# OnurBasci/TransformerBasedNavierStokeSolver

Measured on AMD Instinct MI355X. Metric: ns64_train_samples_per_s, higher is better.
Workload: dtype f32

## Files before the change

### transformerbasednavierstokesolver_amd/csrc/pa2d_gemm.hip

```cpp
#include "pa2d_gemm_common.h"
#include <string.h>


static Pa2dEnv read_env() {
    auto is = [](const char* n, const char* pre) { const char* e = getenv(n); return e && strncmp(e, pre, strlen(pre)) == 0; };
    auto num = [](const char* n, int dflt) { const char* e = getenv(n); return (e && e[0]) ? atoi(e) : dflt; };
    Pa2dEnv v;
    v.conv_halo = is("PA2D_CONV_HALO", "o") ? 0 : (is("PA2D_CONV_HALO", "f") ? 2 : 1);
    v.mc_big_off = is("PA2D_MC_BIG", "o") ? 1 : 0;
    v.kc_bk16 = num("PA2D_KC_BK", 0) == 16 ? 1 : 0;
    v.mc_bk = num("PA2D_MC_BK", 16) == 32 ? 32 : 16;
    v.mc_splits = num("PA2D_MC_SPLITS", 0);
    v.mcb_splits = num("PA2D_MCB_SPLITS", 0);
    v.lin_dw_split = is("PA2D_LIN_DW_SPLIT", "of") ? 0 : 1;
    v.lin_panel = is("PA2D_LIN_PANEL", "of") ? 0 : 1;
    v.lin_rowpanel = is("PA2D_LIN_ROWPANEL", "of") ? 0 : 1;
    v.lin_small_split = is("PA2D_LIN_SMALL_SPLIT", "of") ? 0 : 1;
    v.conv_mfma16 = num("PA2D_CONV_MFMA", 16) == 32 ? 0 : 1;
    v.split_big = num("PA2D_SPLIT_BIG", 1);
    v.slice_map = is("PA2D_SLICE_MAP", "l") ? 0 : 1;
    v.default_engine = is("PA2D_GEMM", "f") ? 0 : (is("PA2D_GEMM", "b") ? 2 : 1);
    return v;
}
static Pa2dEnv g_env = read_env();
const Pa2dEnv& pa2d_env() { return g_env; }
static int kc_bk(bool im2col, int Cin) {
    if (im2col && pa2d_env().kc_bk16) return 16;
    return (!im2col || (Cin % 32) == 0) ? 32 : 16;
}
KCTile kc_tile(int M, int N, bool im2col, int Cin) {
    const int tiles_m = ceil_div(M, 128);
    const long long t128 = (long long)tiles_m * ceil_div(N, 128);
    const long long t12864 = (long long)tiles_m * ceil_div(N, 64);
    const int bk = kc_bk(im2col, Cin);
    if (N > 64 && t128 >= 384) return {128, 128, bk};
    if (t12864 >= 384 || M <= 64) return {128, 64, bk};
    return {64, 64, bk};
}
bool use_split(int engine, int N, bool im2col, int Cin) {
    const int m = engine;
    if (m == 1) return im2col && N > 64 && (Cin % 32) == 0;
    if (m == 2) return N > 64 && (!im2col || (Cin % 32) == 0);
    return false;
}

int launch_kc(const KCParams& p_in, bool im2col, hipStream_t st, hipEvent_t ev0, hipEvent_t ev1) {
    KCParams p = p_in;
    if (!engine_ok(p.engine)) return PA2D_ERR_ARG;
    if (p.M <= 0 || p.N <= 0 || p.K <= 0) return PA2D_OK;
    if (!p.bias2) p.bias_split = 0x7fffffff;
    {
        const unsigned long long ab = ((unsigned long long)(p.M - 1) * p.lda + (im2col ? p.Cin : p.K)) * 4ull;
        const unsigned long long bb = ((unsigned long long)(p.N - 1) * p.ldb + p.K) * 4ull;
        if (ab >= 0xFFFFFFF0ull || bb >= 0xFFFFFFF0ull) return PA2D_ERR_UNSUPPORTED;
        p.a_bytes = (unsigned)ab;
        p.b_bytes = (unsigned)bb;
        const unsigned long long es = p.io_bf16 ? 2ull : 4ull;
        const unsigned long long cb = ((unsigned long long)(p.M - 1) * p.ldc + p.N) * es;
        const unsigned long long rb = p.res ? ((unsigned long long)(p.M - 1) * p.ldres + p.N) * es : 0ull;
        const unsigned long long xb = p.aux ? ((unsigned long long)(p.M - 1) * p.ldaux + p.N) * es : 0ull;
        if (cb >= 0xFFFFFFF0ull || rb >= 0xFFFFFFF0ull || xb >= 0xFFFFFFF0ull) return PA2D_ERR_UNSUPPORTED;
        p.c_bytes = (unsigned)cb; p.res_bytes = (unsigned)rb; p.aux_bytes = (unsigned)xb;
    }
    if ((p.K & 3) || (p.lda & 3) || (p.ldb & 3)) return PA2D_ERR_ARG;
    if (im2col && ((p.Cin & 15) || p.K != (p.taps == 27 ? 27 : 9) * p.Cin)) return PA2D_ERR_UNSUPPORTED;
    if (im2col && (p.epi != 0 || p.res)) return PA2D_ERR_ARG;
    if (ev0 && hipEventRecord(ev0, st) != hipSuccess) return PA2D_ERR_ARG;
    int rc;
    if (!im2col && p.wimg && rowpanel_applies(p)) {
        if (p.wsrc) {
            rc = launch_pack_weight_image(p.wsrc, p.wsn, p.wsk, p.wimg, p.N, p.K, st);
            if (rc) return rc;
        }
        KCParams pp = p;
        pp.M = p.M - p.M % 128;
        rc = launch_kc_rowpanel(pp, p.wimg, st);
        if (!rc && pp.M < p.M) {
            KCParams pt = p_in;
            pt.wimg = nullptr;
            pt.M = p.M - pp.M;
            pt.A = p.A + (size_t)pp.M * p.lda;
            pt.C = p.C + (size_t)pp.M * p.ldc;
            if (p.res) pt.res = p.res + (size_t)pp.M * p.ldres;
            if (p.aux) pt.aux = p.aux + (size_t)pp.M * p.ldaux;
            rc = launch_kc(pt, false, st);
        }
    } else if (panel_applies(p, im2col)) {
        KCParams pp = p;
        pp.M = p.M - p.M % 256;
        rc = launch_kc_panel(pp, st);
        if (!rc && pp.M < p.M) {
            KCParams pt = p_in;
            const size_t ea = p.io_bf16 ? 2 : 4, es = p.io_bf16 ? 2 : 4;
            pt.M = p.M - pp.M;
            pt.A = (const float*)((const char*)p.A + (size_t)pp.M * p.lda * ea);
            pt.C = (float*)((char*)p.C + (size_t)pp.M * p.ldc * es);
            if (p.res) pt.res = (const float*)((const char*)p.res + (size_t)pp.M * p.ldres * es);
            if (p.aux) pt.aux = (float*)((char*)p.aux + (size_t)pp.M * p.ldaux * es);
            rc = launch_kc(pt, false, st);
        }
    } else if (p.io_bf16 || use_split(p.engine, p.N, im2col, p.Cin)) rc = launch_kc_split(p, im2col, st);
// ... 198 lines not shown
```

### transformerbasednavierstokesolver_amd/csrc/pa2d_gemm_mc_planes.hip

```cpp
#include "pa2d_gemm_common.h"
#include "pa2d_bf16_split.h"

struct MCPlanesParams {
    const void* PA; int chA;
    const void* PB; int chB;
    float* slab;
    int Mi, Nj, Mk, chunks_per_split, splits, H, W, Cin;
    unsigned a_bytes, b_bytes;
    int taps;
    long long lda, ldb;
    float* colsum;
};

__device__ __forceinline__ unsigned img_off(int row, int ch) {
    return 256u * row + 16u * (ch ^ (((row & 3) << 2) | ((row >> 2) & 3)));
}

template <int NT, int KS, bool F32SRC = false>
__global__ __launch_bounds__(256, 2) void gemm_mc_planes_kernel(const MCPlanesParams p) {
    constexpr int PIMG = 4096;
    constexpr int STAGE = 2 * NT * KS * PIMG;
    constexpr int NP = 2 * NT * KS;
    __shared__ __attribute__((aligned(16))) unsigned char smem[2 * STAGE];

    const int tid = threadIdx.x, lane = tid & 63, wave = tid >> 6;
    const int tiles_i = (p.Mi + 127) / 128, tiles_j = (p.Nj + 127) / 128;
    int tj, ti, split;
    {
        const int tiles = tiles_i * tiles_j;
        if ((p.splits & 7) == 0) {
            const int xcd = blockIdx.x & 7, slot = blockIdx.x >> 3, q = p.splits >> 3;
            split = xcd * q + slot / tiles;
            const int t = slot % tiles;
            tj = t % tiles_j;
            ti = t / tiles_j;
        } else {
            tj = blockIdx.x % tiles_j;
            ti = (blockIdx.x / tiles_j) % tiles_i;
            split = blockIdx.x / tiles;
        }
    }
    const int wm = wave >> 1, wn = wave & 1;
    const int total_chunks = (p.Mk + 15) / 16;
    const int c_begin = split * p.chunks_per_split;
    const int c_end = min(total_chunks, c_begin + p.chunks_per_split);

    const int j0 = tj * 128, tap = j0 / p.Cin, cb0 = (j0 - tap * p.Cin) >> 5, ca0 = (ti * 128) >> 5;
    const int tap_dy = tap / 3 - 1, tap_dx = tap - (tap / 3) * 3 - 1, tap_shift = tap_dy * p.W + tap_dx;
    const int HW = p.H * p.W;

    const __amdgpu_buffer_rsrc_t ra_rsrc = __builtin_amdgcn_make_buffer_rsrc(const_cast<void*>(p.PA), 0, p.a_bytes, 0x00020000);
    const __amdgpu_buffer_rsrc_t rb_rsrc = __builtin_amdgcn_make_buffer_rsrc(const_cast<void*>(p.PB), 0, p.b_bytes, 0x00020000);

    int s_row[NP];
    unsigned s_goff[NP], s_lds[NP];
    bool s_isb[NP];
#pragma unroll
    for (int s = 0; s < NP; ++s) {
        const int q = tid + 256 * s;
        const int op = q / (256 * NT * KS), r = q - op * (256 * NT * KS);
        const int row = r / (16 * NT), rr = r - row * (16 * NT);
        const int c = rr / (4 * NT), pp = rr - c * (4 * NT);
        const int plane = pp >> 2, piece = pp & 3;
        s_row[s] = row;
        s_isb[s] = op != 0;
        s_goff[s] = (unsigned)((((op ? cb0 : ca0) + c) * NT + plane) * 64 + piece * 16);
        s_lds[s] = (unsigned)(((op * NT + plane) * KS + (row >> 4)) * PIMG) + img_off(row & 15, c * 4 + piece);
    }
    u32x4 rg[F32SRC ? 4 * KS : NP];
    const int frow = tid >> 4, fc8 = tid & 15;
    const unsigned flds = img_off(frow, fc8);
    const bool fok_a = ti * 128 + fc8 * 8 < p.Mi, fok_b = tj * 128 + fc8 * 8 < p.Nj;
    const unsigned fcol_a = (unsigned)(ti * 128 + fc8 * 8) * 4u, fcol_b = (unsigned)(tj * 128 + fc8 * 8) * 4u;
    const unsigned fpitch_a = (unsigned)p.lda * 4u, fpitch_b = (unsigned)p.ldb * 4u;
    float cs[8];
#pragma unroll
    for (int e = 0; e < 8; ++e) cs[e] = 0.f;
#define MP_LOAD(c_)                                                                                       \
    if constexpr (F32SRC) {                                                                               \
        _Pragma("unroll") for (int ks = 0; ks < KS; ++ks) {                                               \
            const int m_ = ((c_) + ks) * 16 + frow;                                                       \
            const bool okr_ = m_ < p.Mk && (c_) + ks < c_end;                                             \
            const unsigned oa_ = (okr_ && fok_a) ? (unsigned)m_ * fpitch_a + fcol_a : OOB_OFF;            \
            const unsigned ob_ = (okr_ && fok_b) ? (unsigned)m_ * fpitch_b + fcol_b : OOB_OFF;            \
            rg[ks * 4 + 0] = __builtin_amdgcn_raw_buffer_load_b128(ra_rsrc, oa_, 0, 0);                   \
            rg[ks * 4 + 1] = __builtin_amdgcn_raw_buffer_load_b128(ra_rsrc, oa_ == OOB_OFF ? OOB_OFF : oa_ + 16u, 0, 0); \
            rg[ks * 4 + 2] = __builtin_amdgcn_raw_buffer_load_b128(rb_rsrc, ob_, 0, 0);                   \
            rg[ks * 4 + 3] = __builtin_amdgcn_raw_buffer_load_b128(rb_rsrc, ob_ == OOB_OFF ? OOB_OFF : ob_ + 16u, 0, 0); \
        }                                                                                                 \
    } else {                                                                                              \
        const int m0_ = (c_) * 16;                                                                        \
        _Pragma("unroll") for (int s = 0; s < NP; ++s) {                                                  \
            const int m_ = m0_ + s_row[s];                                                                \
            bool ok_ = m_ < p.Mk && (KS == 1 || (c_) + (s_row[s] >> 4) < c_end);    \
            int mm_ = m_;                                                                                 \
            if (s_isb[s]) {                                                                               \
                const int n_ = m_ % HW;                                                                   \
                const int y_ = n_ / p.W, x_ = n_ - y_ * p.W;                                              \
                ok_ = ok_ && (unsigned)(y_ + tap_dy) < (unsigned)p.H && (unsigned)(x_ + tap_dx) < (unsigned)p.W; \
                mm_ = m_ + tap_shift;                                                                     \
            }                                                                                             \
            const unsigned rowb_ = (unsigned)mm_ * (unsigned)((s_isb[s] ? p.chB : p.chA) * NT * 64);      \
            rg[s] = s_isb[s] ? __builtin_amdgcn_raw_buffer_load_b128(rb_rsrc, ok_ ? rowb_ + s_goff[s] : OOB_OFF, 0, 0) \
                             : __builtin_amdgcn_raw_buffer_load_b128(ra_rsrc, ok_ ? rowb_ + s_goff[s] : OOB_OFF, 0, 0); \
        }                                                                                                 \
    }
#define MP_STORE(buf_)                                                                                    \
    if constexpr (F32SRC) {                                                                               \
        _Pragma("unroll") for (int ks = 0; ks < KS; ++ks) _Pragma("unroll") for (int op = 0; op < 2; ++op) { \
            const u32x4 u0_ = rg[ks * 4 + op * 2], u1_ = rg[ks * 4 + op * 2 + 1];                         \
            const float4 v0_ = make_float4(__uint_as_float(u0_.x), __uint_as_float(u0_.y), __uint_as_float(u0_.z), __uint_as_float(u0_.w)); \
            const float4 v1_ = make_float4(__uint_as_float(u1_.x), __uint_as_float(u1_.y), __uint_as_float(u1_.z), __uint_as_float(u1_.w)); \
            if (op == 0 && do_cs) {                                                                       \
                cs[0] += v0_.x; cs[1] += v0_.y; cs[2] += v0_.z; cs[3] += v0_.w;                           \
                cs[4] += v1_.x; cs[5] += v1_.y; cs[6] += v1_.z; cs[7] += v1_.w;                           \
            }                                                                                             \
            bf16x4 h0_, m0_, l0_, h1_, m1_, l1_;                                                          \
            split3(v0_, h0_, m0_, l0_);                                                                   \
            split3(v1_, h1_, m1_, l1_);                                                                   \
            unsigned char* d_ = smem + (buf_) * STAGE + flds;                                             \
            *reinterpret_cast<bf16x8*>(d_ + ((op * NT + 0) * KS + ks) * PIMG) = __builtin_shufflevector(h0_, h1_, 0, 1, 2, 3, 4, 5, 6, 7); \
            if (NT == 3) {                                                                                \
                *reinterpret_cast<bf16x8*>(d_ + ((op * NT + 1) * KS + ks) * PIMG) = __builtin_shufflevector(m0_, m1_, 0, 1, 2, 3, 4, 5, 6, 7); \
                *reinterpret_cast<bf16x8*>(d_ + ((op * NT + 2) * KS + ks) * PIMG) = __builtin_shufflevector(l0_, l1_, 0, 1, 2, 3, 4, 5, 6, 7); \
            }                                                                                             \
        }                                                                                                 \
    } else {                                                                                              \
        _Pragma("unroll") for (int s = 0; s < NP; ++s)                                                    \
            *reinterpret_cast<u32x4*>(smem + (buf_) * STAGE + s_lds[s]) = rg[s];                          \
    }
    const bool do_cs = F32SRC && p.colsum != nullptr && tj == 0;

    f32x16 acc[2][2];
#pragma unroll
    for (int i = 0; i < 2; ++i)
#pragma unroll
        for (int j = 0; j < 2; ++j)
#pragma unroll
            for (int r = 0; r < 16; ++r) acc[i][j][r] = 0.f;

    const int g = lane >> 4, q4 = (lane & 15) >> 2, pq = lane & 3;
    unsigned fa[2][2], fb[2][2];
#pragma unroll
    for (int t = 0; t < 2; ++t)
#pragma unroll
        for (int r = 0; r < 2; ++r) {
            const int row = 8 * (g >> 1) + 4 * r + q4;
            const int cha = ((wm * 64 + t * 32) >> 3) + 2 * (g & 1) + (pq >> 1);
            const int chb = ((wn * 64 + t * 32) >> 3) + 2 * (g & 1) + (pq >> 1);
            fa[t][r] = img_off(row, cha) + 8u * (pq & 1);
            fb[t][r] = img_off(row, chb) + 8u * (pq & 1);
        }

    if (c_begin < c_end) {
        MP_LOAD(c_begin)
        MP_STORE(0)
    }
    __syncthreads();
    for (int c = c_begin; c < c_end; c += KS) {
        const int buf = ((c - c_begin) / KS) & 1;
        if (c + KS < c_end) { MP_LOAD(c + KS) }
#pragma unroll
        for (int ks = 0; ks < KS; ++ks) {
        const unsigned char* st = smem + buf * STAGE + ks * PIMG;
        bf16x8 af[2][NT], bf[2][NT];
#pragma unroll
        for (int t = 0; t < 2; ++t)
#pragma unroll
            for (int pl = 0; pl < NT; ++pl) {
                typedef __attribute__((address_space(3))) s16x4 lds_s16x4;
                const s16x4 a0 = __builtin_amdgcn_ds_read_tr16_b64_v4i16((lds_s16x4*)(st + pl * KS * PIMG + fa[t][0]));
                const s16x4 a1 = __builtin_amdgcn_ds_read_tr16_b64_v4i16((lds_s16x4*)(st + pl * KS * PIMG + fa[t][1]));
                const s16x4 b0 = __builtin_amdgcn_ds_read_tr16_b64_v4i16((lds_s16x4*)(st + (NT + pl) * KS * PIMG + fb[t][0]));
                const s16x4 b1 = __builtin_amdgcn_ds_read_tr16_b64_v4i16((lds_s16x4*)(st + (NT + pl) * KS * PIMG + fb[t][1]));
                const s16x8 av = __builtin_shufflevector(a0, a1, 0, 1, 2, 3, 4, 5, 6, 7);
                const s16x8 bv = __builtin_shufflevector(b0, b1, 0, 1, 2, 3, 4, 5, 6, 7);
                af[t][pl] = __builtin_bit_cast(bf16x8, av);
                bf[t][pl] = __builtin_bit_cast(bf16x8, bv);
            }
#pragma unroll
        for (int i = 0; i < 2; ++i)
#pragma unroll
            for (int j = 0; j < 2; ++j) {
                if constexpr (NT == 3) {
                    acc[i][j] = __builtin_amdgcn_mfma_f32_32x32x16_bf16(af[i][1], bf[j][1], acc[i][j], 0, 0, 0);
                    acc[i][j] = __builtin_amdgcn_mfma_f32_32x32x16_bf16(af[i][2], bf[j][0], acc[i][j], 0, 0, 0);
                    acc[i][j] = __builtin_amdgcn_mfma_f32_32x32x16_bf16(af[i][0], bf[j][2], acc[i][j], 0, 0, 0);
                    acc[i][j] = __builtin_amdgcn_mfma_f32_32x32x16_bf16(af[i][1], bf[j][0], acc[i][j], 0, 0, 0);
                    acc[i][j] = __builtin_amdgcn_mfma_f32_32x32x16_bf16(af[i][0], bf[j][1], acc[i][j], 0, 0, 0);
                }
                acc[i][j] = __builtin_amdgcn_mfma_f32_32x32x16_bf16(af[i][0], bf[j][0], acc[i][j], 0, 0, 0);
            }
        }
        if (c + KS < c_end) { MP_STORE(buf ^ 1) }
        __syncthreads();
    }
#undef MP_LOAD
#undef MP_STORE

    if constexpr (F32SRC) {
        if (do_cs) {
            float* sm = reinterpret_cast<float*>(smem);
#pragma unroll
            for (int e = 0; e < 8; ++e) sm[frow * 128 + fc8 * 8 + e] = cs[e];
            __syncthreads();
            if (tid < 128) {
                float t = 0.f;
#pragma unroll
                for (int r = 0; r < 16; ++r) t += sm[r * 128 + tid];
                if (ti * 128 + tid < p.Mi) p.colsum[(size_t)split * p.Mi + ti * 128 + tid] = t;
            }
        }
    }
    float* out = p.slab + (size_t)split * p.Mi * p.Nj;
    const int col0 = tj * 128 + wn * 64 + (lane & 31);
    const int row0 = ti * 128 + wm * 64 + 4 * (lane >> 5);
#pragma unroll
    for (int j = 0; j < 2; ++j)
#pragma unroll
        for (int i = 0; i < 2; ++i)
#pragma unroll
            for (int r = 0; r < 16; ++r) {
                const int row = row0 + i * 32 + (r & 3) + 8 * (r >> 2);
                if (!F32SRC || (row < p.Mi && col0 + j * 32 < p.Nj)) out[(size_t)row * p.Nj + col0 + j * 32] = acc[i][j][r];
            }
}

bool mc_planes_supported(int C, int Cin) { return (C % 64) == 0 && (Cin % 128) == 0; }

int launch_mc_planes(const void* PA, const void* PB, int C, int Cin, int Mk, int H, int W, float* slab,
                     const MCPlan& pl, int NT, hipStream_t st) {
    if (!mc_planes_supported(C, Cin) || !pl.big) return PA2D_ERR_UNSUPPORTED;
    MCPlanesParams p;
    p.PA = PA; p.chA = 2 * C / 32; p.PB = PB; p.chB = Cin / 32; p.slab = slab;
    p.Mi = 2 * C; p.Nj = 9 * Cin; p.Mk = Mk; p.chunks_per_split = pl.chunks_per_split; p.splits = pl.splits;
    p.H = H; p.W = W; p.Cin = Cin; p.taps = 9;
    const unsigned long long ab = (unsigned long long)Mk * p.chA * NT * 64, bb = (unsigned long long)Mk * p.chB * NT * 64;
    if (ab >= 0xFFFFFFF0ull || bb >= 0xFFFFFFF0ull) return PA2D_ERR_UNSUPPORTED;
    p.a_bytes = (unsigned)ab; p.b_bytes = (unsigned)bb;
    const dim3 grid((p.Mi / 128) * (p.Nj / 128) * pl.splits);
    if (NT == 3) hipLaunchKernelGGL((gemm_mc_planes_kernel<3, 1>), grid, dim3(256), 0, st, p);
    else hipLaunchKernelGGL((gemm_mc_planes_kernel<1, 4>), grid, dim3(256), 0, st, p);
    PA2D_CHECK_LAUNCH();
    return PA2D_OK;
}

template <int NT, int KS>
__global__ __launch_bounds__(512, 1) void gemm_mc_planes_big_kernel(const MCPlanesParams p, const int per_xcd) {
    constexpr int PIMG = 8192;
    constexpr int STAGE = 2 * NT * KS * PIMG;
    constexpr int NP = (2 * NT * KS * 512) / 512;
    extern __shared__ __attribute__((aligned(16))) unsigned char smem[];

    const int tid = threadIdx.x, lane = tid & 63, wave = tid >> 6;
    const int tiles_i = (p.Mi + 255) / 256, tiles_j = (p.Nj + 255) / 256;
    const int tiles = tiles_i * tiles_j;
    const int lin = (blockIdx.x & 7) * per_xcd + (blockIdx.x >> 3);
    if ((int)(blockIdx.x >> 3) >= per_xcd || lin >= tiles * p.splits) return;
    const int split = lin / tiles, t_ = lin - split * tiles;
    const int ti = t_ / tiles_j, tj = t_ - ti * tiles_j;
    const int wm = wave >> 2, wn = wave & 3;
    const int total_chunks = (p.Mk + 15) / 16;
    const int c_begin = split * p.chunks_per_split;
    const int c_end = min(total_chunks, c_begin + p.chunks_per_split);
    const int HW = p.taps == 1 ? 1 : p.H * p.W;

    const __amdgpu_buffer_rsrc_t ra_rsrc = __builtin_amdgcn_make_buffer_rsrc(const_cast<void*>(p.PA), 0, p.a_bytes, 0x00020000);
    const __amdgpu_buffer_rsrc_t rb_rsrc = __builtin_amdgcn_make_buffer_rsrc(const_cast<void*>(p.PB), 0, p.b_bytes, 0x00020000);

    const int row16 = tid >> 5, cgrp = (tid & 31) >> 2, piece = tid & 3;
    const bool colok_a = ti * 256 + cgrp * 32 < p.Mi;
    const unsigned goff_a = (unsigned)((((ti * 256) >> 5) + cgrp) * NT * 64 + piece * 16);
    const int jc = tj * 256 + cgrp * 32;
    const int tap = p.taps == 1 ? 4 : jc / p.Cin;
    const bool colok_b = jc < p.Nj;
    const unsigned goff_b = (unsigned)((p.taps == 1 ? (jc >> 5) : ((jc - tap * p.Cin) >> 5)) * NT * 64 + piece * 16);
    const int tap_dy = tap / 3 - 1, tap_dx = tap - (tap / 3) * 3 - 1, tap_shift = tap_dy * p.W + tap_dx;
    const unsigned pitch_a = (unsigned)(p.chA * NT * 64), pitch_b = (unsigned)(p.chB * NT * 64);
    const unsigned lds_off = 512u * row16 + 16u * ((unsigned)(cgrp * 4 + piece) ^ (unsigned)(((row16 & 3) << 2) | ((row16 >> 2) & 3)));
#define MB_LOAD(c_, RG)                                                                                   \
    {                                                                                                     \
        _Pragma("unroll") for (int ks = 0; ks < KS; ++ks) {                                               \
            const int m_ = ((c_) + ks) * 16 + row16;                                                      \
            const bool okr_ = m_ < p.Mk && (c_) + ks < c_end;             \
            bool okb_ = okr_ && colok_b;                                                                  \
            int mm_ = m_;                                                                                 \
            if (p.taps != 1) {       \
                okb_ = okb_ && (unsigned)(ly + tap_dy) < (unsigned)p.H && (unsigned)(lx + tap_dx) < (unsigned)p.W; \
                mm_ = m_ + tap_shift;                                                                     \
                lx += 16;                                                                                 \
                while (lx >= p.W) { lx -= p.W; ++ly; }                                                    \
                while (ly >= p.H) ly -= p.H;                                                              \
            }                                                                                             \
            const unsigned oa_ = (okr_ && colok_a) ? (unsigned)m_ * pitch_a + goff_a : OOB_OFF;           \
            const unsigned ob_ = okb_ ? (unsigned)mm_ * pitch_b + goff_b : OOB_OFF;                       \
            _Pragma("unroll") for (int pl = 0; pl < NT; ++pl) {                                           \
                RG[pl * KS + ks] = __builtin_amdgcn_raw_buffer_load_b128(ra_rsrc, oa_ == OOB_OFF ? OOB_OFF : oa_ + pl * 64u, 0, 0); \
                RG[(NT + pl) * KS + ks] = __builtin_amdgcn_raw_buffer_load_b128(rb_rsrc, ob_ == OOB_OFF ? OOB_OFF : ob_ + pl * 64u, 0, 0); \
            }                                                                                             \
        }                                                                                                 \
    }
#define MB_STORE(buf_, RG)                                                                                \
    {                                                                                                     \
        _Pragma("unroll") for (int s = 0; s < NP; ++s)                                                    \
            *reinterpret_cast<u32x4*>(smem + (buf_) * STAGE + s * PIMG + lds_off) = RG[s];                \
    }
    u32x4 rg0[NP];
    int ly = 0, lx = 0;
    if (p.taps != 1) {
        const int n0 = (c_begin * 16 + row16) % HW;
        ly = n0 / p.W;
        lx = n0 - ly * p.W;
    }

    f32x16 acc[4][2];
#pragma unroll
    for (int i = 0; i < 4; ++i)
#pragma unroll
        for (int j = 0; j < 2; ++j)
#pragma unroll
            for (int r = 0; r < 16; ++r) acc[i][j][r] = 0.f;

    const int g = lane >> 4, q4 = (lane & 15) >> 2, pq = lane & 3;
    unsigned fa[4][2], fb[2][2];
#pragma unroll
    for (int r = 0; r < 2; ++r) {
        const int row = 8 * (g >> 1) + 4 * r + q4;
        const unsigned swz = (unsigned)(((row & 3) << 2) | ((row >> 2) & 3));
#pragma unroll
        for (int t = 0; t < 4; ++t) {
            const int cha = ((wm * 128 + t * 32) >> 3) + 2 * (g & 1) + (pq >> 1);
            fa[t][r] = 512u * row + 16u * ((unsigned)cha ^ swz) + 8u * (pq & 1);
        }
#pragma unroll
        for (int t = 0; t < 2; ++t) {
            const int chb = ((wn * 64 + t * 32) >> 3) + 2 * (g & 1) + (pq >> 1);
            fb[t][r] = 512u * row + 16u * ((unsigned)chb ^ swz) + 8u * (pq & 1);
        }
    }

#define MB_COMPUTE(buf_)                                                                                  \
    _Pragma("unroll") for (int ks = 0; ks < KS; ++ks) {                                                   \
        const unsigned char* st = smem + (buf_) * STAGE + ks * PIMG;                                      \
        bf16x8 af[4][NT], bf[2][NT];                                                                      \
        typedef __attribute__((address_space(3))) s16x4 lds_s16x4;                                        \
        _Pragma("unroll") for (int pl = 0; pl < NT; ++pl) {                                               \
            _Pragma("unroll") for (int t = 0; t < 4; ++t) {                                               \
                const s16x4 a0 = __builtin_amdgcn_ds_read_tr16_b64_v4i16((lds_s16x4*)(st + pl * KS * PIMG + fa[t][0])); \
                const s16x4 a1 = __builtin_amdgcn_ds_read_tr16_b64_v4i16((lds_s16x4*)(st + pl * KS * PIMG + fa[t][1])); \
                af[t][pl] = __builtin_bit_cast(bf16x8, __builtin_shufflevector(a0, a1, 0, 1, 2, 3, 4, 5, 6, 7)); \
            }                                                                                             \
            _Pragma("unroll") for (int t = 0; t < 2; ++t) {                                               \
                const s16x4 b0 = __builtin_amdgcn_ds_read_tr16_b64_v4i16((lds_s16x4*)(st + (NT + pl) * KS * PIMG + fb[t][0])); \
                const s16x4 b1 = __builtin_amdgcn_ds_read_tr16_b64_v4i16((lds_s16x4*)(st + (NT + pl) * KS * PIMG + fb[t][1])); \
                bf[t][pl] = __builtin_bit_cast(bf16x8, __builtin_shufflevector(b0, b1, 0, 1, 2, 3, 4, 5, 6, 7)); \
            }                                                                                             \
        }                                                                                                 \
        _Pragma("unroll") for (int i = 0; i < 4; ++i)                                                     \
            _Pragma("unroll") for (int j = 0; j < 2; ++j) {                                               \
                if constexpr (NT == 3) {                                        \
                    acc[i][j] = __builtin_amdgcn_mfma_f32_32x32x16_bf16(af[i][1], bf[j][1], acc[i][j], 0, 0, 0); \
                    acc[i][j] = __builtin_amdgcn_mfma_f32_32x32x16_bf16(af[i][2], bf[j][0], acc[i][j], 0, 0, 0); \
                    acc[i][j] = __builtin_amdgcn_mfma_f32_32x32x16_bf16(af[i][0], bf[j][2], acc[i][j], 0, 0, 0); \
                    acc[i][j] = __builtin_amdgcn_mfma_f32_32x32x16_bf16(af[i][1], bf[j][0], acc[i][j], 0, 0, 0); \
                    acc[i][j] = __builtin_amdgcn_mfma_f32_32x32x16_bf16(af[i][0], bf[j][1], acc[i][j], 0, 0, 0); \
                }                                                                                         \
                acc[i][j] = __builtin_amdgcn_mfma_f32_32x32x16_bf16(af[i][0], bf[j][0], acc[i][j], 0, 0, 0); \
            }                                                                                             \
    }
    if (c_begin < c_end) {
        MB_LOAD(c_begin, rg0)
        MB_STORE(0, rg0)
        if (c_begin + KS < c_end) MB_LOAD(c_begin + KS, rg0)
    }
    __syncthreads();
    for (int c = c_begin; c < c_end; c += KS) {
        const int buf = ((c - c_begin) / KS) & 1;
        if (c + KS < c_end) {
            MB_STORE(buf ^ 1, rg0)
            if (c + 2 * KS < c_end) MB_LOAD(c + 2 * KS, rg0)
        }
        MB_COMPUTE(buf)
        __syncthreads();
    }
#undef MB_COMPUTE
#undef MB_LOAD
#undef MB_STORE

    float* out = p.slab + (size_t)split * p.Mi * p.Nj;
    const int col0 = tj * 256 + wn * 64 + (lane & 31);
    const int row0 = ti * 256 + wm * 128 + 4 * (lane >> 5);
#pragma unroll
    for (int j = 0; j < 2; ++j) {
        const int col = col0 + j * 32;
        if (col >= p.Nj) continue;
#pragma unroll
        for (int i = 0; i < 4; ++i)
#pragma unroll
            for (int r = 0; r < 16; ++r) {
                const int row = row0 + i * 32 + (r & 3) + 8 * (r >> 2);
                if (row < p.Mi) out[(size_t)row * p.Nj + col] = acc[i][j][r];
            }
    }
}

MCPlan plan_mc_planes_big(int Mi, int Nj, int Mk) {
    MCPlan pl;
    if (Mk < 1) Mk = 1;
    pl.big = 2;
    const int tiles = ceil_div(Mi, 256) * ceil_div(Nj, 256);
    const int total_chunks = ceil_div(Mk, 16);
    int splits = 256 / tiles;
    if (pa2d_env().mcb_splits > 0) splits = pa2d_env().mcb_splits;
    const int max_splits = total_chunks / 8 > 0 ? total_chunks / 8 : 1;
    if (splits > max_splits) splits = max_splits;
    if (splits < 1) splits = 1;
    pl.chunks_per_split = ceil_div(total_chunks, splits);
    pl.splits = ceil_div(total_chunks, pl.chunks_per_split);
    pl.slab_floats = (size_t)pl.splits * Mi * Nj;
    return pl;
}

bool mc_planes_big_applies(int C, int Cin, int Mk) {
    if (pa2d_env().mc_big_off) return false;
    return (C % 16) == 0 && (Cin % 32) == 0 && 2 * C >= 256 && 9 * Cin >= 256 && Mk >= 16 * 8 * 4;
}

int launch_mc_planes_big(const void* PA, const void* PB, int C, int Cin, int Mk, int H, int W, float* slab,
                         const MCPlan& pl, int NT, hipStream_t st) {
    return launch_mc_planes_big_raw(PA, 2 * C, PB, Cin, 9, Mk, H, W, slab, pl, NT, st);
}

int launch_mc_planes_big_raw(const void* PA, int Mi, const void* PB, int Cin, int taps, int Mk, int H, int W, float* slab,
                             const MCPlan& pl, int NT, hipStream_t st) {
    if ((Mi & 31) || (Cin & 31) || (taps != 1 && taps != 9)) return PA2D_ERR_UNSUPPORTED;
    MCPlanesParams p;
    p.PA = PA; p.chA = Mi / 32; p.PB = PB; p.chB = Cin / 32; p.slab = slab;
    p.Mi = Mi; p.Nj = taps * Cin; p.Mk = Mk; p.chunks_per_split = pl.chunks_per_split; p.splits = pl.splits;
    p.H = H; p.W = W; p.Cin = Cin; p.taps = taps;
    const unsigned long long ab = (unsigned long long)Mk * p.chA * NT * 64, bb = (unsigned long long)Mk * p.chB * NT * 64;
    if (ab >= 0xFFFFFFF0ull || bb >= 0xFFFFFFF0ull) return PA2D_ERR_UNSUPPORTED;
    p.a_bytes = (unsigned)ab; p.b_bytes = (unsigned)bb;
    const int wgs = ceil_div(p.Mi, 256) * ceil_div(p.Nj, 256) * pl.splits;
    const int per_xcd = ceil_div(wgs, 8);
    const dim3 grid(per_xcd * 8);
    if (NT == 3) {
        const int smem = 2 * 2 * 3 * 1 * 8192;
        {
            hipError_t e = hipFuncSetAttribute(reinterpret_cast<const void*>(&gemm_mc_planes_big_kernel<3, 1>),
                                               hipFuncAttributeMaxDynamicSharedMemorySize, smem);
            if (e != hipSuccess) return (int)e;
        }
        hipLaunchKernelGGL((gemm_mc_planes_big_kernel<3, 1>), grid, dim3(512), smem, st, p, per_xcd);
    } else {
        const int smem = 2 * 2 * 1 * 4 * 8192;
        {
            hipError_t e = hipFuncSetAttribute(reinterpret_cast<const void*>(&gemm_mc_planes_big_kernel<1, 4>),
                                               hipFuncAttributeMaxDynamicSharedMemorySize, smem);
            if (e != hipSuccess) return (int)e;
        }
        hipLaunchKernelGGL((gemm_mc_planes_big_kernel<1, 4>), grid, dim3(512), smem, st, p, per_xcd);
    }
    PA2D_CHECK_LAUNCH();
    return PA2D_OK;
}

bool mc_f32src_applies(int Mi, int Nj, int Mk, long long lda, long long ldb) {
    return pa2d_env().lin_dw_split && (Mi % 8) == 0 && (Nj % 8) == 0 && Mi > 64 && Nj > 64 && Mk >= 16 * 8 * 16 && (lda % 4) == 0 && (ldb % 4) == 0;
}

int launch_mc_f32src(const float* A, long long lda, int Mi, const float* B, long long ldb, int Nj, int Mk, float* slab,
                     const MCPlan& pl, int NT, float* colsum, hipStream_t st) {
    if (!pl.big) return PA2D_ERR_UNSUPPORTED;
    MCPlanesParams p = {};
    p.PA = A; p.PB = B; p.slab = slab; p.lda = lda; p.ldb = ldb; p.colsum = colsum;
    p.Mi = Mi; p.Nj = Nj; p.Mk = Mk; p.chunks_per_split = pl.chunks_per_split; p.splits = pl.splits;
    p.H = 1; p.W = 1; p.Cin = Nj; p.taps = 1; p.chA = 0; p.chB = 0;
    const unsigned long long ab = ((unsigned long long)(Mk - 1) * lda + Mi) * 4ull, bb = ((unsigned long long)(Mk - 1) * ldb + Nj) * 4ull;
    if (ab >= 0xFFFFFFF0ull || bb >= 0xFFFFFFF0ull) return PA2D_ERR_UNSUPPORTED;
    p.a_bytes = (unsigned)ab; p.b_bytes = (unsigned)bb;
    const dim3 grid(ceil_div(Mi, 128) * ceil_div(Nj, 128) * pl.splits);
    if (NT == 3) hipLaunchKernelGGL((gemm_mc_planes_kernel<3, 1, true>), grid, dim3(256), 0, st, p);
    else hipLaunchKernelGGL((gemm_mc_planes_kernel<1, 4, true>), grid, dim3(256), 0, st, p);
    PA2D_CHECK_LAUNCH();
    return PA2D_OK;
}
```

### transformerbasednavierstokesolver_amd/csrc/pa2d_internal.h

```cpp
#pragma once
#include <hip/hip_runtime.h>
#include <stdint.h>

typedef float f32x16 __attribute__((ext_vector_type(16)));
typedef float f32x4 __attribute__((ext_vector_type(4)));

#define PA2D_OK 0
#define PA2D_ERR_ARG 1001
#define PA2D_ERR_UNSUPPORTED 1002
#define PA2D_ERR_WORKSPACE 1003

#define PA2D_CHECK_LAUNCH()                         \
    do {                                            \
        hipError_t e__ = hipGetLastError();         \
        if (e__ != hipSuccess) return (int)e__;     \
    } while (0)

enum { ACT_NONE = 0, ACT_GELU = 1, ACT_TANH = 2, ACT_SIGMOID = 3, ACT_RELU = 4, ACT_SOFTPLUS = 5,
       ACT_ELU = 6, ACT_SILU = 7 };

__device__ __forceinline__ float normal_cdf(float x, float& e_out) {
#pragma clang fp contract(off)
    const float z = fabsf(x) * 0.70710678118654752440f;
    const float t = __builtin_amdgcn_rcpf(fmaf(0.3275911f, z, 1.0f));
// ... 16 lines not shown
    float e;
    const float cdf = normal_cdf(x, e);
    return fmaf(x * 0.39894228040143267794f, e, cdf);
}

__device__ __forceinline__ float act_fwd(int id, float x) {
    switch (id) {
        case ACT_GELU: return gelu_exact(x);
        case ACT_TANH: return tanhf(x);
        case ACT_SIGMOID: return 1.0f / (1.0f + expf(-x));
        case ACT_RELU: return x > 0.f ? x : 0.f;
        case ACT_SOFTPLUS: return x > 20.f ? x : log1pf(expf(x));
        case ACT_ELU: return x > 0.f ? x : expm1f(x);
        case ACT_SILU: return x / (1.0f + expf(-x));
        default: return x;
    }
}

__device__ __forceinline__ float act_bwd(int id, float x) {
    switch (id) {
        case ACT_GELU: return dgelu_exact(x);
        case ACT_TANH: { const float t = tanhf(x); return 1.0f - t * t; }
        case ACT_SIGMOID: { const float s = 1.0f / (1.0f + expf(-x)); return s * (1.0f - s); }
        case ACT_RELU: return x > 0.f ? 1.f : 0.f;
        case ACT_SOFTPLUS: return x > 20.f ? 1.f : 1.0f / (1.0f + expf(-x));
        case ACT_ELU: return x > 0.f ? 1.f : expf(x);
        case ACT_SILU: { const float s = 1.0f / (1.0f + expf(-x)); return s * (1.0f + x * (1.0f - s)); }
        default: return 1.f;
    }
}

__device__ __forceinline__ float wave_sum(float v) {
#pragma unroll
    for (int o = 32; o > 0; o >>= 1) v += __shfl_xor(v, o, 64);
    return v;
}
__device__ __forceinline__ float wave_max(float v) {
#pragma unroll
    for (int o = 32; o > 0; o >>= 1) v = fmaxf(v, __shfl_xor(v, o, 64));
    return v;
}

typedef unsigned int u32x4 __attribute__((ext_vector_type(4)));
#define OOB_OFF 0xFFFFFFFFu

__device__ __forceinline__ __amdgpu_buffer_rsrc_t make_rsrc(const float* base, unsigned bytes) {
    return __builtin_amdgcn_make_buffer_rsrc(const_cast<float*>(base), 0, bytes, 0x00020000);
}
__device__ __forceinline__ float4 buf_load4(__amdgpu_buffer_rsrc_t r, unsigned voff) {
    const u32x4 v = __builtin_amdgcn_raw_buffer_load_b128(r, voff, 0, 0);
    return make_float4(__uint_as_float(v.x), __uint_as_float(v.y), __uint_as_float(v.z), __uint_as_float(v.w));
}


__device__ __forceinline__ float buf_load1(__amdgpu_buffer_rsrc_t r, unsigned voff) {
    return __uint_as_float(__builtin_amdgcn_raw_buffer_load_b32(r, voff, 0, 0));
}
__device__ __forceinline__ void buf_store1(__amdgpu_buffer_rsrc_t r, unsigned voff, float v) {
    __builtin_amdgcn_raw_buffer_store_b32(__float_as_uint(v), r, voff, 0, 0);
}

__device__ __forceinline__ float2 buf_load2(__amdgpu_buffer_rsrc_t r, unsigned voff) {
    typedef unsigned int u32x2_ __attribute__((ext_vector_type(2)));
    const u32x2_ v = __builtin_amdgcn_raw_buffer_load_b64(r, voff, 0, 0);
    return make_float2(__uint_as_float(v.x), __uint_as_float(v.y));
}
__device__ __forceinline__ void buf_store4(__amdgpu_buffer_rsrc_t r, unsigned voff, float4 v) {
    u32x4 u = {__float_as_uint(v.x), __float_as_uint(v.y), __float_as_uint(v.z), __float_as_uint(v.w)};
    __builtin_amdgcn_raw_buffer_store_b128(u, r, voff, 0, 0);
}

#define PA2D_ACT_SAVE_DERIVATIVE_BIT 0x100

struct Pa2dEnv {
    int conv_halo;
    int mc_big_off;
    int kc_bk16;
    int mc_bk;
    int mc_splits;
    int mcb_splits;
    int lin_dw_split;
    int lin_panel;
    int conv_mfma16;
    int lin_small_split;
    int lin_rowpanel;
    int split_big;
    int slice_map;
    int default_engine;
};
const Pa2dEnv& pa2d_env();

static inline int pa2d_zero(void* p, size_t bytes, hipStream_t st) {
    if (!p || !bytes) return PA2D_OK;
    return (int)hipMemsetAsync(p, 0, bytes, st);
}
static inline int ceil_div(int a, int b) { return (a + b - 1) / b; }
static inline long long ceil_div_ll(long long a, long long b) { return (a + b - 1) / b; }

struct ReduceSegs { int nseg; long long begin[5]; float* dst[4]; };
int pa2d_launch_reduce_segs(const float* slab, int nslab, long long count, const ReduceSegs& segs, int accumulate,
                            hipStream_t st);

typedef __bf16 bf16_t;
template <typename T> struct Act;
template <> struct Act<float> {
    static constexpr unsigned ES = 4;
    static __device__ __forceinline__ float4 ld4(const float* p) { return *reinterpret_cast<const float4*>(p); }
    static __device__ __forceinline__ void st4(float* p, float4 v) { *reinterpret_cast<float4*>(p) = v; }
    static __device__ __forceinline__ float ld1(const float* p) { return *p; }
    static __device__ __forceinline__ float4 bld4(__amdgpu_buffer_rsrc_t r, unsigned off) { return buf_load4(r, off); }
    static __device__ __forceinline__ float2 bld2(__amdgpu_buffer_rsrc_t r, unsigned off) { return buf_load2(r, off); }
    static __device__ __forceinline__ float bld1(__amdgpu_buffer_rsrc_t r, unsigned off) { return buf_load1(r, off); }
    static __device__ __forceinline__ float bld1s(__amdgpu_buffer_rsrc_t r, unsigned off, unsigned soff) {
        return __uint_as_float(__builtin_amdgcn_raw_buffer_load_b32(r, off, soff, 0));
    }
    static __device__ __forceinline__ void bst4(__amdgpu_buffer_rsrc_t r, unsigned off, float4 v) { buf_store4(r, off, v); }
    static __device__ __forceinline__ void bst1(__amdgpu_buffer_rsrc_t r, unsigned off, float v) { buf_store1(r, off, v); }
};
__device__ __forceinline__ float bf16_bits_to_f32(unsigned short b) { return __uint_as_float((unsigned)b << 16); }
__device__ __forceinline__ unsigned short f32_to_bf16_bits(float x) {
    const bf16_t h = (bf16_t)x;
    return __builtin_bit_cast(unsigned short, h);
}
__device__ __forceinline__ unsigned pack_bf16x2(float lo, float hi) {
    return (unsigned)f32_to_bf16_bits(lo) | ((unsigned)f32_to_bf16_bits(hi) << 16);
}
template <> struct Act<bf16_t> {
    static constexpr unsigned ES = 2;
    static __device__ __forceinline__ float4 unpack4(uint2 q) {
        return make_float4(__uint_as_float(q.x << 16), __uint_as_float(q.x & 0xFFFF0000u), __uint_as_float(q.y << 16),
                           __uint_as_float(q.y & 0xFFFF0000u));
    }
    static __device__ __forceinline__ float4 ld4(const bf16_t* p) { return unpack4(*reinterpret_cast<const uint2*>(p)); }
    static __device__ __forceinline__ void st4(bf16_t* p, float4 v) {
        *reinterpret_cast<uint2*>(p) = make_uint2(pack_bf16x2(v.x, v.y), pack_bf16x2(v.z, v.w));
    }
    static __device__ __forceinline__ float ld1(const bf16_t* p) { return (float)*p; }
    static __device__ __forceinline__ float4 bld4(__amdgpu_buffer_rsrc_t r, unsigned off) {
        typedef unsigned int u32x2_ __attribute__((ext_vector_type(2)));
        const u32x2_ q = __builtin_amdgcn_raw_buffer_load_b64(r, off, 0, 0);
        return unpack4(make_uint2(q.x, q.y));
    }
    static __device__ __forceinline__ float2 bld2(__amdgpu_buffer_rsrc_t r, unsigned off) {
        const unsigned q = __builtin_amdgcn_raw_buffer_load_b32(r, off, 0, 0);
        return make_float2(__uint_as_float(q << 16), __uint_as_float(q & 0xFFFF0000u));
    }
    static __device__ __forceinline__ float bld1(__amdgpu_buffer_rsrc_t r, unsigned off) {
        return bf16_bits_to_f32(__builtin_amdgcn_raw_buffer_load_b16(r, off, 0, 0));
    }
    static __device__ __forceinline__ float bld1s(__amdgpu_buffer_rsrc_t r, unsigned off, unsigned soff) {
        return bf16_bits_to_f32(__builtin_amdgcn_raw_buffer_load_b16(r, off, soff, 0));
    }
    static __device__ __forceinline__ void bst4(__amdgpu_buffer_rsrc_t r, unsigned off, float4 v) {
        typedef unsigned int u32x2_ __attribute__((ext_vector_type(2)));
        const u32x2_ q = {pack_bf16x2(v.x, v.y), pack_bf16x2(v.z, v.w)};
        __builtin_amdgcn_raw_buffer_store_b64(q, r, off, 0, 0);
    }
    static __device__ __forceinline__ void bst1(__amdgpu_buffer_rsrc_t r, unsigned off, float v) {
        __builtin_amdgcn_raw_buffer_store_b16(f32_to_bf16_bits(v), r, off, 0, 0);
    }
};
__device__ __forceinline__ __amdgpu_buffer_rsrc_t make_rsrc_v(const void* base, unsigned bytes) {
    return __builtin_amdgcn_make_buffer_rsrc(const_cast<void*>(base), 0, bytes, 0x00020000);
}

__device__ __forceinline__ bool slice_decode(int xcd_map, int B, int heads, int nchunk, int& b, int& hh, int& chunk, int& bid) {
// ... 22 lines not shown
```

Before: 69.51.

## Use 16x16x32 MFMA with triple-buffered LDS in split-bf16 multi-chunk weight-gradient kernels

Adds a 16x16x32 bf16 MFMA variant of the split-precision (3-plane bf16) multi-chunk GEMM kernels, used for linear and conv weight gradients. It switches operand fragment loads to transposed LDS reads and moves from two to three LDS buffers, so loads, f32-to-bf16 split conversion and stores overlap the MFMA chain more deeply. The variant is on by default for the NT==3 path when the output slab is 16-byte aligned, and can be turned off with an environment variable. It raises LDS use per block, which may lower occupancy, and it adds a large new code path whose fragment indexing must be correct.

```diff
diff --git a/transformerbasednavierstokesolver_amd/csrc/pa2d_gemm.hip b/transformerbasednavierstokesolver_amd/csrc/pa2d_gemm.hip
--- a/transformerbasednavierstokesolver_amd/csrc/pa2d_gemm.hip
+++ b/transformerbasednavierstokesolver_amd/csrc/pa2d_gemm.hip
@@ -17,6 +17,7 @@
     v.lin_rowpanel = is("PA2D_LIN_ROWPANEL", "of") ? 0 : 1;
     v.lin_small_split = is("PA2D_LIN_SMALL_SPLIT", "of") ? 0 : 1;
     v.conv_mfma16 = num("PA2D_CONV_MFMA", 16) == 32 ? 0 : 1;
+    v.mc_mfma16 = num("PA2D_MC_MFMA", 16) == 32 ? 0 : 1;
     v.split_big = num("PA2D_SPLIT_BIG", 1);
     v.slice_map = is("PA2D_SLICE_MAP", "l") ? 0 : 1;
     v.default_engine = is("PA2D_GEMM", "f") ? 0 : (is("PA2D_GEMM", "b") ? 2 : 1);
diff --git a/transformerbasednavierstokesolver_amd/csrc/pa2d_gemm_mc_planes.hip b/transformerbasednavierstokesolver_amd/csrc/pa2d_gemm_mc_planes.hip
--- a/transformerbasednavierstokesolver_amd/csrc/pa2d_gemm_mc_planes.hip
+++ b/transformerbasednavierstokesolver_amd/csrc/pa2d_gemm_mc_planes.hip
@@ -16,12 +16,12 @@
     return 256u * row + 16u * (ch ^ (((row & 3) << 2) | ((row >> 2) & 3)));
 }
 
-template <int NT, int KS, bool F32SRC = false>
+template <int NT, int KS, bool F32SRC = false, bool MF16 = false>
 __global__ __launch_bounds__(256, 2) void gemm_mc_planes_kernel(const MCPlanesParams p) {
     constexpr int PIMG = 4096;
     constexpr int STAGE = 2 * NT * KS * PIMG;
     constexpr int NP = 2 * NT * KS;
-    __shared__ __attribute__((aligned(16))) unsigned char smem[2 * STAGE];
+    __shared__ __attribute__((aligned(16))) unsigned char smem[(MF16 ? 3 : 2) * STAGE];
 
     const int tid = threadIdx.x, lane = tid & 63, wave = tid >> 6;
     const int tiles_i = (p.Mi + 127) / 128, tiles_j = (p.Nj + 127) / 128;
@@ -131,6 +131,139 @@
     }
     const bool do_cs = F32SRC && p.colsum != nullptr && tj == 0;
 
+    if constexpr (MF16) {
+        static_assert(NT == 3 && KS == 1 && F32SRC, "the 16x16x32 form is written for the split engine's linear weight gradient");
+        f32x4 acc[4][4];
+#pragma unroll
+        for (int i = 0; i < 4; ++i)
+#pragma unroll
+            for (int j = 0; j < 4; ++j) acc[i][j] = f32x4{0.f, 0.f, 0.f, 0.f};
+        const int kq = lane >> 4, q4 = (lane & 15) >> 2, pq = lane & 3;
+        unsigned fa[2], fb[2];
+#pragma unroll
+        for (int r = 0; r < 2; ++r) {
+            const int row = 8 * (kq & 1) + 4 * r + q4;
+            fa[r] = img_off(row, wm * 8 + (pq >> 1)) + 8u * (pq & 1);
+            fb[r] = img_off(row, wn * 8 + (pq >> 1)) + 8u * (pq & 1);
+        }
+        typedef __attribute__((address_space(3))) s16x4 lds_s16x4;
+#define MP16_FRAG(base_, t_, pl_)                                                                         \
+    __builtin_bit_cast(bf16x8, __builtin_shufflevector(                                                   \
+        __builtin_amdgcn_ds_read_tr16_b64_v4i16((lds_s16x4*)(smem + ((base_[0] ^ ((unsigned)(t_) << 5)) + (pl_) * PIMG))), \
+        __builtin_amdgcn_ds_read_tr16_b64_v4i16((lds_s16x4*)(smem + ((base_[1] ^ ((unsigned)(t_) << 5)) + (pl_) * PIMG))), \
+        0, 1, 2, 3, 4, 5, 6, 7))
+#define MP16_MMA(ib_, AF)                                                                                 \
+    _Pragma("unroll") for (int j = 0; j < 4; ++j) {        \
+        acc[ib_][j] = __builtin_amdgcn_mfma_f32_16x16x32_bf16(xf[j][1], AF[1], acc[ib_][j], 0, 0, 0);     \
+        acc[ib_][j] = __builtin_amdgcn_mfma_f32_16x16x32_bf16(xf[j][0], AF[2], acc[ib_][j], 0, 0, 0);     \
+        acc[ib_][j] = __builtin_amdgcn_mfma_f32_16x16x32_bf16(xf[j][2], AF[0], acc[ib_][j], 0, 0, 0);     \
+        acc[ib_][j] = __builtin_amdgcn_mfma_f32_16x16x32_bf16(xf[j][0], AF[1], acc[ib_][j], 0, 0, 0);     \
+        acc[ib_][j] = __builtin_amdgcn_mfma_f32_16x16x32_bf16(xf[j][1], AF[0], acc[ib_][j], 0, 0, 0);     \
+        acc[ib_][j] = __builtin_amdgcn_mfma_f32_16x16x32_bf16(xf[j][0], AF[0], acc[ib_][j], 0, 0, 0);     \
+    }
+        bf16x8 pk[2][NT];
+#define MP16_CONVERT()                                                                                    \
+    _Pragma("unroll") for (int op = 0; op < 2; ++op) {                                                    \
+        const u32x4 u0_ = rg[op * 2], u1_ = rg[op * 2 + 1];                                               \
+        const float4 v0_ = make_float4(__uint_as_float(u0_.x), __uint_as_float(u0_.y), __uint_as_float(u0_.z), __uint_as_float(u0_.w)); \
+        const float4 v1_ = make_float4(__uint_as_float(u1_.x), __uint_as_float(u1_.y), __uint_as_float(u1_.z), __uint_as_float(u1_.w)); \
+        if (op == 0 && do_cs) {                                                                           \
+            cs[0] += v0_.x; cs[1] += v0_.y; cs[2] += v0_.z; cs[3] += v0_.w;                               \
+            cs[4] += v1_.x; cs[5] += v1_.y; cs[6] += v1_.z; cs[7] += v1_.w;                               \
+        }                                                                                                 \
+        bf16x4 h0_, m0_, l0_, h1_, m1_, l1_;                                                              \
+        split3(v0_, h0_, m0_, l0_);                                                                       \
+        split3(v1_, h1_, m1_, l1_);                                                                       \
+        pk[op][0] = __builtin_shufflevector(h0_, h1_, 0, 1, 2, 3, 4, 5, 6, 7);                            \
+        pk[op][1] = __builtin_shufflevector(m0_, m1_, 0, 1, 2, 3, 4, 5, 6, 7);                            \
+        pk[op][2] = __builtin_shufflevector(l0_, l1_, 0, 1, 2, 3, 4, 5, 6, 7);                            \
+    }
+#define MP16_WRITE(buf_)                                                                                  \
+    _Pragma("unroll") for (int op = 0; op < 2; ++op) _Pragma("unroll") for (int pl = 0; pl < NT; ++pl)    \
+        *reinterpret_cast<bf16x8*>(smem + (buf_) * STAGE + flds + (op * NT + pl) * PIMG) = pk[op][pl];
+        const int nst = c_end - c_begin, steps = (nst + 1) >> 1;
+        if (nst > 0) {
+            MP_LOAD(c_begin)
+            MP16_CONVERT()
+            MP16_WRITE(0)
+            MP_LOAD(c_begin + 1)
+            MP16_CONVERT()
+            MP16_WRITE(1)
+            if (steps > 1) { MP_LOAD(c_begin + 2) }
+        }
+        __syncthreads();
+        int sp = 0, sq = 1, sr = 2;
+        for (int k = 0; k < steps; ++k) {
+            const bool has_next = k + 1 < steps;
+            const unsigned lo = (unsigned)((kq >> 1) ? sq : sp) * (unsigned)STAGE;
+            const unsigned ua[2] = {fa[0] + lo, fa[1] + lo};
+            const unsigned ub[2] = {fb[0] + lo + NT * PIMG, fb[1] + lo + NT * PIMG};
+            bf16x8 xf[4][NT];
+#pragma unroll
+            for (int j = 0; j < 4; ++j)
+#pragma unroll
+                for (int pl = 0; pl < NT; ++pl) xf[j][pl] = MP16_FRAG(ub, j, pl);
+            bf16x8 afc[NT], afn[NT];
+#pragma unroll
+            for (int pl = 0; pl < NT; ++pl) afc[pl] = MP16_FRAG(ua, 0, pl);
+#pragma unroll
+            for (int ib = 0; ib < 4; ++ib) {
+                if (ib < 3) {
+#pragma unroll
+                    for (int pl = 0; pl < NT; ++pl) afn[pl] = MP16_FRAG(ua, ib + 1, pl);
+                }
+                if (ib == 1 && has_next) {
+                    MP16_CONVERT()
+                    MP16_WRITE(sr)
+                    MP_LOAD(c_begin + 2 * k + 3)
+                }
+                if (ib == 3) {
+                    if (has_next) {
+                        MP16_CONVERT()
+                        if (k + 2 < steps) { MP_LOAD(c_begin + 2 * k + 4) }
+                    }
+                    __syncthreads();
+                    if (has_next) { MP16_WRITE(sp) }
+                }
+                MP16_MMA(ib, afc)
+#pragma unroll
+                for (int pl = 0; pl < NT; ++pl) afc[pl] = afn[pl];
+            }
+            __syncthreads();
+            const int t = sp;
+            sp = sr;
+            sr = sq;
+            sq = t;
+        }
+#undef MP16_CONVERT
+#undef MP16_WRITE
+#undef MP16_MMA
+#undef MP16_FRAG
+        if (do_cs) {
+            float* sm = reinterpret_cast<float*>(smem);
+#pragma unroll
+            for (int e = 0; e < 8; ++e) sm[frow * 128 + fc8 * 8 + e] = cs[e];
+            __syncthreads();
+            if (tid < 128) {
+                float t = 0.f;
+#pragma unroll
+                for (int r = 0; r < 16; ++r) t += sm[r * 128 + tid];
+                if (ti * 128 + tid < p.Mi) p.colsum[(size_t)split * p.Mi + ti * 128 + tid] = t;
+            }
+        }
+        float* out = p.slab + (size_t)split * p.Mi * p.Nj;
+#pragma unroll
+        for (int j = 0; j < 4; ++j) {
+            const int col = tj * 128 + wn * 64 + j * 16 + 4 * kq;
+#pragma unroll
+            for (int ib = 0; ib < 4; ++ib) {
+                const int row = ti * 128 + wm * 64 + ib * 16 + (lane & 15);
+                if (row < p.Mi && col < p.Nj) *reinterpret_cast<f32x4*>(out + (size_t)row * p.Nj + col) = acc[ib][j];
+            }
+        }
+        return;
+    }
+
     f32x16 acc[2][2];
 #pragma unroll
     for (int i = 0; i < 2; ++i)
@@ -245,7 +378,7 @@
     return PA2D_OK;
 }
 
-template <int NT, int KS>
+template <int NT, int KS, bool MF16 = false>
 __global__ __launch_bounds__(512, 1) void gemm_mc_planes_big_kernel(const MCPlanesParams p, const int per_xcd) {
     constexpr int PIMG = 8192;
     constexpr int STAGE = 2 * NT * KS * PIMG;
@@ -313,6 +446,100 @@
         lx = n0 - ly * p.W;
     }
 
+    if constexpr (MF16) {
+        static_assert(NT == 3 && KS == 1, "the 16x16x32 form is written for the split engine");
+        f32x4 acc[8][4];
+#pragma unroll
+        for (int i = 0; i < 8; ++i)
+#pragma unroll
+            for (int j = 0; j < 4; ++j) acc[i][j] = f32x4{0.f, 0.f, 0.f, 0.f};
+        const int kq = lane >> 4, q4 = (lane & 15) >> 2, pq = lane & 3;
+        unsigned fa[2], fb[2];
+#pragma unroll
+        for (int r = 0; r < 2; ++r) {
+            const int row = 8 * (kq & 1) + 4 * r + q4;
+            const unsigned swz = (unsigned)(((row & 3) << 2) | ((row >> 2) & 3));
+            fa[r] = 512u * row + 16u * ((unsigned)(wm * 16 + (pq >> 1)) ^ swz) + 8u * (pq & 1);
+            fb[r] = 512u * row + 16u * ((unsigned)(wn * 8 + (pq >> 1)) ^ swz) + 8u * (pq & 1);
+        }
+        typedef __attribute__((address_space(3))) s16x4 lds_s16x4;
+#define MB16_FRAG(base_, t_, pl_)                                                                         \
+    __builtin_bit_cast(bf16x8, __builtin_shufflevector(                                                   \
+        __builtin_amdgcn_ds_read_tr16_b64_v4i16((lds_s16x4*)(smem + ((base_[0] ^ ((unsigned)(t_) << 5)) + (pl_) * PIMG))), \
+        __builtin_amdgcn_ds_read_tr16_b64_v4i16((lds_s16x4*)(smem + ((base_[1] ^ ((unsigned)(t_) << 5)) + (pl_) * PIMG))), \
+        0, 1, 2, 3, 4, 5, 6, 7))
+#define MB16_MMA(ib_, AF)                                                                                 \
+    _Pragma("unroll") for (int j = 0; j < 4; ++j) {        \
+        acc[ib_][j] = __builtin_amdgcn_mfma_f32_16x16x32_bf16(xf[j][1], AF[1], acc[ib_][j], 0, 0, 0);     \
+        acc[ib_][j] = __builtin_amdgcn_mfma_f32_16x16x32_bf16(xf[j][0], AF[2], acc[ib_][j], 0, 0, 0);     \
+        acc[ib_][j] = __builtin_amdgcn_mfma_f32_16x16x32_bf16(xf[j][2], AF[0], acc[ib_][j], 0, 0, 0);     \
+        acc[ib_][j] = __builtin_amdgcn_mfma_f32_16x16x32_bf16(xf[j][0], AF[1], acc[ib_][j], 0, 0, 0);     \
+        acc[ib_][j] = __builtin_amdgcn_mfma_f32_16x16x32_bf16(xf[j][1], AF[0], acc[ib_][j], 0, 0, 0);     \
+        acc[ib_][j] = __builtin_amdgcn_mfma_f32_16x16x32_bf16(xf[j][0], AF[0], acc[ib_][j], 0, 0, 0);     \
+    }
+        const int nst = c_end - c_begin, steps = (nst + 1) >> 1;
+        if (nst > 0) {
+            MB_LOAD(c_begin, rg0)
+            MB_STORE(0, rg0)
+            MB_LOAD(c_begin + 1, rg0)
+            MB_STORE(1, rg0)
+            if (steps > 1) MB_LOAD(c_begin + 2, rg0)
+        }
+        __syncthreads();
+        int sp = 0, sq = 1, sr = 2;
+        for (int k = 0; k < steps; ++k) {
+            const unsigned lo = (unsigned)((kq >> 1) ? sq : sp) * (unsigned)STAGE;
+            const unsigned ua[2] = {fa[0] + lo, fa[1] + lo};
+            const unsigned ub[2] = {fb[0] + lo + NT * PIMG, fb[1] + lo + NT * PIMG};
+            bf16x8 xf[4][NT];
+#pragma unroll
+            for (int j = 0; j < 4; ++j)
+#pragma unroll
+                for (int pl = 0; pl < NT; ++pl) xf[j][pl] = MB16_FRAG(ub, j, pl);
+            bf16x8 afc[NT], afn[NT];
+#pragma unroll
+            for (int pl = 0; pl < NT; ++pl) afc[pl] = MB16_FRAG(ua, 0, pl);
+#pragma unroll
+            for (int ib = 0; ib < 8; ++ib) {
+                if (ib < 7) {
+#pragma unroll
+                    for (int pl = 0; pl < NT; ++pl) afn[pl] = MB16_FRAG(ua, ib + 1, pl);
+                }
+                if (ib == 4) {
+                    MB_STORE(sr, rg0)
+                    MB_LOAD(c_begin + 2 * k + 3, rg0)
+                }
+                if (ib == 7) {
+                    __syncthreads();
+                    MB_STORE(sp, rg0)
+                    MB_LOAD(c_begin + 2 * k + 4, rg0)
+                }
+                MB16_MMA(ib, afc)
+#pragma unroll
+                for (int pl = 0; pl < NT; ++pl) afc[pl] = afn[pl];
+            }
+            __syncthreads();
+            const int t = sp;
+            sp = sr;
+            sr = sq;
+            sq = t;
+        }
+#undef MB16_MMA
+#undef MB16_FRAG
+        float* out = p.slab + (size_t)split * p.Mi * p.Nj;
+#pragma unroll
+        for (int j = 0; j < 4; ++j) {
+            const int col = tj * 256 + wn * 64 + j * 16 + 4 * kq;
+            if (col >= p.Nj) continue;
+#pragma unroll
+            for (int ib = 0; ib < 8; ++ib) {
+                const int row = ti * 256 + wm * 128 + ib * 16 + (lane & 15);
+                if (row < p.Mi) *reinterpret_cast<f32x4*>(out + (size_t)row * p.Nj + col) = acc[ib][j];
+            }
+        }
+        return;
+    }
+
     f32x16 acc[4][2];
 #pragma unroll
     for (int i = 0; i < 4; ++i)
@@ -444,7 +671,15 @@
     const int wgs = ceil_div(p.Mi, 256) * ceil_div(p.Nj, 256) * pl.splits;
     const int per_xcd = ceil_div(wgs, 8);
     const dim3 grid(per_xcd * 8);
-    if (NT == 3) {
+    if (NT == 3 && pa2d_env().mc_mfma16 && (reinterpret_cast<uintptr_t>(slab) & 15) == 0) {
+        const int smem = 3 * 2 * 3 * 1 * 8192;
+        {
+            hipError_t e = hipFuncSetAttribute(reinterpret_cast<const void*>(&gemm_mc_planes_big_kernel<3, 1, true>),
+                                               hipFuncAttributeMaxDynamicSharedMemorySize, smem);
+            if (e != hipSuccess) return (int)e;
+        }
+        hipLaunchKernelGGL((gemm_mc_planes_big_kernel<3, 1, true>), grid, dim3(512), smem, st, p, per_xcd);
+    } else if (NT == 3) {
         const int smem = 2 * 2 * 3 * 1 * 8192;
         {
             hipError_t e = hipFuncSetAttribute(reinterpret_cast<const void*>(&gemm_mc_planes_big_kernel<3, 1>),
@@ -480,7 +715,9 @@
     if (ab >= 0xFFFFFFF0ull || bb >= 0xFFFFFFF0ull) return PA2D_ERR_UNSUPPORTED;
     p.a_bytes = (unsigned)ab; p.b_bytes = (unsigned)bb;
     const dim3 grid(ceil_div(Mi, 128) * ceil_div(Nj, 128) * pl.splits);
-    if (NT == 3) hipLaunchKernelGGL((gemm_mc_planes_kernel<3, 1, true>), grid, dim3(256), 0, st, p);
+    if (NT == 3 && pa2d_env().mc_mfma16 && (Nj % 4) == 0 && (reinterpret_cast<uintptr_t>(slab) & 15) == 0)
+        hipLaunchKernelGGL((gemm_mc_planes_kernel<3, 1, true, true>), grid, dim3(256), 0, st, p);
+    else if (NT == 3) hipLaunchKernelGGL((gemm_mc_planes_kernel<3, 1, true>), grid, dim3(256), 0, st, p);
     else hipLaunchKernelGGL((gemm_mc_planes_kernel<1, 4, true>), grid, dim3(256), 0, st, p);
     PA2D_CHECK_LAUNCH();
     return PA2D_OK;
diff --git a/transformerbasednavierstokesolver_amd/csrc/pa2d_internal.h b/transformerbasednavierstokesolver_amd/csrc/pa2d_internal.h
--- a/transformerbasednavierstokesolver_amd/csrc/pa2d_internal.h
+++ b/transformerbasednavierstokesolver_amd/csrc/pa2d_internal.h
@@ -122,6 +122,7 @@
     int lin_dw_split;
     int lin_panel;
     int conv_mfma16;
+    int mc_mfma16;
     int lin_small_split;
     int lin_rowpanel;
     int split_big;
```

Result: faster. 70.46 (median of 6 runs) (+1.4%).
